# rlglab/minizero

Hardware: AMD Instinct MI355X
Metric: self-play leaf-evals/s (9x9 Go AlphaZero n=400) (higher is better)
Workload: dtype f32; 1 GPU; BASELINE configs[1]: 9x9 Go AlphaZero, n=400, 6 blocks x 64 ch, 256 parallel games per GPU, synthetic fixed-weight net (seed 0), Dirichlet noise + random rotation + softmax-count moves (reference defaults); games_per_gpu=256, actor_num_simulation=400, pipeline_lanes=1, backend=nccl

## Files before the change

minizero_amd/csrc/pool_body.h:

```cpp
#pragma once
#include "pool.h"
#include <cfloat>
#include <climits>

#ifndef MZ_LPROF
#define MZ_LPROF(k)
#endif

namespace mz {

__device__ __forceinline__ float normalizedMean(const PoolView& v, float reward, float mean, float cnt, int player, int bsize, float lo, float hi)
{
    float value = reward + v.gamma * mean;
    if (v.value_rescale) {
        if (bsize < 2) { return 1.0f; }
        value = (value - lo) / (hi - lo);
        value = 2 * value - 1;
        value = value < -1.0f ? -1.0f : value;
        value = value > 1.0f ? 1.0f : value;
    }
    value = (player == v.flipping_player) ? -value : value;
    return (value * cnt - 0.0f) / (cnt + 0.0f);
}

// ... 83 lines not shown
typedef __attribute__((address_space(3))) const float LdsCFloat;
typedef __attribute__((address_space(3))) const double LdsCDbl;
constexpr int kSpecCap = 128;
constexpr int kSpecWay = 4 + 3 * kSpecCap;
constexpr int kGw = 4, kLv = 64 / kGw;
#ifndef MZ_SPEC_WAYS
#define MZ_SPEC_WAYS 16
#endif
constexpr int kSpecWays = MZ_SPEC_WAYS;
#define MZ_SPEC_WAYS_IS(n) static_assert(mz::kSpecWays == (n), "this translation unit sizes its LDS for " #n " remembered paths (pool_body.h MZ_SPEC_WAYS)")
static_assert((kSpecWays & (kSpecWays - 1)) == 0 && kSpecWays >= 2 && kSpecWays <= 64, "a power of two of at most one wave's lanes");
constexpr int kHelpSegs = 3;
constexpr int kHelpHdr = 16;
constexpr int kHelpSeg = kHelpHdr + 4 * kLv;
enum : int {
    kSpecNext = kSpecWays * kSpecWay,
    kSpecPasses = kSpecNext + 1,
    kSpecFound = kSpecNext + 3,
    kSpecLevels = kSpecNext + 5,
    kSpecLastWay = kSpecNext + 6,
    kSpecHelped = kSpecNext + 7,
    kSpecHelp = kSpecNext + 8,
};
constexpr int kSpecWords = kSpecHelp + kHelpSegs * kHelpSeg;
constexpr int kSpecNode = 4, kSpecFc = 4 + kSpecCap, kSpecNc = 4 + 2 * kSpecCap;
struct SpecMem { LdsI32* w; LdsCFloat* bias; LdsCDbl* sqrt; };

struct SpecStage {
    double* sqrt_w;
    float* bias_w;
    int* spec_w;
    __device__ __forceinline__ SpecMem mem(bool walk) const { return SpecMem{walk ? (LdsI32*)spec_w : nullptr, (LdsCFloat*)bias_w, (LdsCDbl*)sqrt_w}; }
    __device__ __forceinline__ float* end() const { return reinterpret_cast<float*>(spec_w + kSpecWords); }
};
template <class View>
__device__ __forceinline__ SpecStage specStage(const View& pv, double* rcp_w, int rcp_n, int tid)
{
    const int tab_n = rcp_n - 2;
    double* sqrt_w = rcp_w + rcp_n;
    float* bias_w = reinterpret_cast<float*>(sqrt_w + tab_n);
    int* spec_w = reinterpret_cast<int*>(bias_w + tab_n + (tab_n & 1));
    for (int i = tid; i < tab_n; i += 512) { sqrt_w[i] = pv.sqrt_tab[i]; bias_w[i] = pv.bias_tab[i]; }
    if (tid < kSpecWays) { spec_w[tid * kSpecWay] = 0; }
    if (tid < 8) { spec_w[kSpecNext + tid] = 0; }
    if (tid < kHelpSegs) { spec_w[kSpecHelp + tid * kHelpSeg] = 0; }
    return SpecStage{sqrt_w, bias_w, spec_w};
}

struct SelectJoin {
    LdsI32* word;
    LdsI32* stats;
    int want, leaf, poll_limit, code;
    int* err;
};

template <bool SPEC = false, bool JOIN = false, class RcpPtr>
__device__ __forceinline__ void selectBody(const PoolView& v, const int* __restrict__ start, int g, int lane, RcpPtr rcp, SpecMem sm = SpecMem{nullptr, nullptr, nullptr}, int serial = 0,
                                           SelectJoin join = SelectJoin{nullptr, nullptr, 0, -1, 0, 0, nullptr})
{
    GNodeRec* recs = (GNodeRec*)(v.rec + size_t(g) * v.cap);
    int* path = v.path + size_t(g) * v.max_depth;
    int* pact = v.path_action + size_t(g) * v.max_depth;
    int* hact = v.host_path_action ? v.host_path_action + size_t(g) * v.max_depth : nullptr;
    MZ_GLOBAL const float* bias_tab = (MZ_GLOBAL const float*)v.bias_tab;
    MZ_GLOBAL const double* sqrt_tab = (MZ_GLOBAL const double*)v.sqrt_tab;
    LdsI32* spec = nullptr;
    auto note = [&](int d, int n, const NodeRec& r) {
        if (!SPEC || !sm.w) { return; }
        if (d == 1) {
            const int w = lane < kSpecWays ? lane : 0;
            const int lw = sm.w[w * kSpecWay], nw = sm.w[w * kSpecWay + kSpecNode + 1];
            const unsigned long long m = __ballot(lane < kSpecWays && lw > 1 && nw == n);
            int way;
            if (m != 0) {
                way = static_cast<int>(__builtin_ctzll(m));
                if (lane == 0) { sm.w[kSpecFound] += 1; }
            } else {
                way = __builtin_amdgcn_readfirstlane(sm.w[kSpecNext]) & (kSpecWays - 1);
                if (lane == 0) { sm.w[kSpecNext] = way + 1; sm.w[way * kSpecWay] = 0; }
            }
            spec = sm.w + way * kSpecWay;
            if (lane == 0) { sm.w[kSpecLastWay] = way; }
        }
        if (spec && lane == 0 && d < kSpecCap) {
            spec[kSpecNode + d] = n;
            spec[kSpecFc + d] = r.first_child;
            spec[kSpecNc + d] = r.num_children;
        }
    };
    const int bsize = v.bound_size[g];
    const float lo = v.bound_lo[g], hi = v.bound_hi[g];
    auto uniformRec = [](NodeRec r) {
        NodeRec u;
        u.count = __int_as_float(__builtin_amdgcn_readfirstlane(__float_as_int(r.count)));
        u.mean = __int_as_float(__builtin_amdgcn_readfirstlane(__float_as_int(r.mean)));
        u.policy = __int_as_float(__builtin_amdgcn_readfirstlane(__float_as_int(r.policy)));
        u.reward = __int_as_float(__builtin_amdgcn_readfirstlane(__float_as_int(r.reward)));
        u.first_child = __builtin_amdgcn_readfirstlane(r.first_child);
        u.num_children = __builtin_amdgcn_readfirstlane(r.num_children);
        u.action = __builtin_amdgcn_readfirstlane(r.action);
        u.players = __builtin_amdgcn_readfirstlane(r.players);
        return u;
    };
    NodeRec cur = uniformRec(loadRec(recs));
    int node = 0, depth = 1;
    if (lane == 0) { path[0] = 0; pact[0] = cur.action; if (hact) { hact[0] = cur.action; } }
    const int st = start ? __builtin_amdgcn_readfirstlane(start[g]) : 0;
    if (st > 0) {
        node = st;
        cur = uniformRec(loadRec(recs + st));
        if (lane == 0) { path[1] = st; pact[1] = cur.action; if (hact) { hact[1] = cur.action; } }
// ... 289 lines not shown
            unsigned long long m = __ballot(vis);
            while (m) { const int j = __builtin_ctzll(m); m &= m - 1; sum_of_win += laneF(q, j); sum += 1; }
        }
        const float init_q = v.atari_init_q ? (sum > 0 ? sum_of_win / sum : 1.0f) : (sum_of_win - 1) / (sum + 1);
        float bs = -FLT_MAX, bp = -FLT_MAX;
        int bi = INT_MAX;
        NodeRec best = c0;
        auto consider = [&](const NodeRec& c, float q, int i) {
            const float bpol = bias * c.policy;
            const float value_u = static_cast<float>((static_cast<double>(bpol) * sqrtN) / static_cast<double>(1 + c.count));
            const float value_q = (c.count == 0.0f) ? init_q : q;
            const float score = value_u + value_q;
            if (better(score, c.policy, i, bs, bp, bi)) { bs = score; bp = c.policy; bi = i; best = c; }
        };
        if (has0) { consider(c0, q0, lane); }
        if (has1) { consider(c1, q1, lane + 64); }
        for (int cb = 128; cb < nc; cb += 64) {
            const int i = cb + lane;
            if (i < nc) {
                const NodeRec c = loadRec(recs + fc + i);
                const float q = (c.count != 0.0f) ? normalizedMean(v, c.reward, c.mean, c.count, cplayer, bsize, lo, hi) : 0.0f;
                consider(c, q, i);
            }
        }
        float rs = bs, rp = bp;
        int ri = bi;
        dppBest<0x111, 0xF>(rs, rp, ri);
        dppBest<0x112, 0xF>(rs, rp, ri);
        dppBest<0x114, 0xF>(rs, rp, ri);
        dppBest<0x118, 0xF>(rs, rp, ri);
        dppBest<0x142, 0xA>(rs, rp, ri);
        dppBest<0x143, 0xC>(rs, rp, ri);
        ri = laneI(ri, 63);
        const int owner = __builtin_ctzll(__ballot(bi == ri));
        cur.count = laneF(best.count, owner);
        cur.first_child = laneI(best.first_child, owner);
        cur.num_children = laneI(best.num_children, owner);
        cur.action = laneI(best.action, owner);
        cur.players = laneI(best.players, owner);
        node = fc + ri;
        note(depth, node, cur);
        if (lane == 0) {
            path[depth] = node;
            pact[depth] = cur.action;
            if (hact) { hact[depth] = cur.action; }
        }
        ++depth;
    }
    if (lane == 0) {
        v.path_len[g] = depth;
        if (v.host_path_len) { v.host_path_len[g] = depth; }
        if (spec) { spec[0] = depth < kSpecCap ? depth : kSpecCap; }
    }
}

template <class RcpPtr>
__device__ __forceinline__ void selectSpecHelper(const PoolView& v, int g, int lane, int seg, int serial, RcpPtr rcp, SpecMem sm)
{
    if (!sm.w || v.atari_init_q || v.value_rescale || seg < 1 || seg > kHelpSegs) { return; }
    LdsI32* out = sm.w + kSpecHelp + (seg - 1) * kHelpSeg;
    const int way = __builtin_amdgcn_readfirstlane(sm.w[kSpecLastWay]) & (kSpecWays - 1);
    LdsI32* spec = sm.w + way * kSpecWay;
    const int plen = __builtin_amdgcn_readfirstlane(spec[0]);
    const int L0 = 1 + seg * kLv, depth = L0 + 1;
    const int max_depth = __builtin_amdgcn_readfirstlane(v.max_depth);
    int adv = 0, n0 = -1;
    int f_count = 0, f_fc = 0, f_nc = 0, f_act = 0, f_pl = 0, f_node = 0;
    if (L0 + 1 < plen && L0 + 1 < kSpecCap) {
        GNodeRec* recs = (GNodeRec*)(v.rec + size_t(g) * v.cap);
        MZ_GLOBAL const float* bias_tab = (MZ_GLOBAL const float*)v.bias_tab;
        MZ_GLOBAL const double* sqrt_tab = (MZ_GLOBAL const double*)v.sqrt_tab;
        int K = plen - L0 < kSpecCap - L0 ? plen - L0 : kSpecCap - L0;
        K = K < kLv ? K : kLv;
        const int k = lane / kGw, j = lane % kGw, Lk = L0 + k, base8 = lane - j;
        const bool inrange = k < K;
        n0 = __builtin_amdgcn_readfirstlane(spec[kSpecNode + L0]);
        const int nk = inrange ? spec[kSpecNode + Lk] : 0;
        const int fck = inrange ? spec[kSpecFc + Lk] : 0;
        const int nck = inrange ? spec[kSpecNc + Lk] : 0;
        const int pfc = (inrange && k >= 1) ? spec[kSpecFc + Lk - 1] : 0;
        const int pnc = (inrange && k >= 1) ? spec[kSpecNc + Lk - 1] : 0;
        const int nl = nck < kGw ? nck : kGw;
        const bool ld = inrange && j < nl && fck >= 0 && fck + j < v.cap;
        const NodeRec c = loadRec(recs + (ld ? fck + j : 0));
        const NodeRec h0 = loadRec(recs + ((n0 >= 0 && n0 < v.cap) ? n0 : 0));
        const int idx = nk - pfc;
        const bool idx_ok = idx >= 0 && idx < kGw && idx < pnc;
        const int srcl = idx_ok ? base8 - kGw + idx : lane;
        float hcount = __shfl(c.count, srcl);
        int hfc = __shfl(c.first_child, srcl), hnc = __shfl(c.num_children, srcl), hpl = __shfl(c.players, srcl);
        if (k == 0) { hcount = h0.count; hfc = h0.first_child; hnc = h0.num_children; hpl = h0.players; }
        bool okk = inrange && ld == (j < nl) && nck > 0 && n0 >= 0 && n0 < v.cap && (k == 0 || idx_ok) && hfc == fck && hnc == nck && hcount >= 1.0f;
        int Nk = static_cast<int>(hcount - 1);
        Nk = okk ? Nk : 0;
        const float biask = sm.bias ? sm.bias[Nk] : bias_tab[Nk];
        const double sqrtNk = sm.sqrt ? sm.sqrt[Nk] : sqrt_tab[Nk];
        const unsigned visn = static_cast<unsigned>(hpl) >> 16;
        const int nek = (visn == 0xFFFFu) ? nck : (nck < static_cast<int>(visn) + 1 ? nck : static_cast<int>(visn) + 1);
        okk = okk && nek <= kGw;
        const int cplk = (hpl >> 8) & 0xFF;
        const bool has = okk && j < nek;
        const RcpPtr rp = rcp + (has ? static_cast<int>(c.count) : 0);
        bool tiny = false;
        const LevelEval e = evalChild(v, c, cplk, biask, sqrtNk, rp[0], rp[1], &tiny);
        const bool vis = has && c.count != 0.0f;
        if (__ballot(vis && tiny) == 0) {
// ... 264 lines not shown
```

minizero_amd/csrc/sim.hip:

```cpp
#include "sim_az_body.h"
#include "sim_mz_body.h"

namespace mz {

MZ_SPEC_WAYS_IS(16);

template <int H, int W, int CIN0_PAD, int CDYN_PAD, int CPAD>
__global__ __launch_bounds__(512) void sim_kernel_mz(const SimArgs* __restrict__ a_, int sim0, int nsims, int host_start, int pre_epoch)
{
    CSimArgs* a = (CSimArgs*)a_;
    extern __shared__ __attribute__((aligned(16))) float tiles[];
    const int g = blockIdx.x, tid = threadIdx.x, lane = tid & 63, wave = tid >> 6;
    constexpr int CM = CIN0_PAD > CDYN_PAD ? (CIN0_PAD > CPAD ? CIN0_PAD : CPAD) : (CDYN_PAD > CPAD ? CDYN_PAD : CPAD);
    constexpr int kTileFloats = kTowerTiles * CM * planeStride(H, W);
    double* rcp_w = reinterpret_cast<double*>(tiles + kTileFloats);
    const int rcp_n = a->rcp_n;
    for (int i = tid; i < rcp_n; i += 512) { rcp_w[i] = a->pv.rcp_tab[i]; }
    LdsCDouble* rcp_lds = (LdsCDouble*)rcp_w;
    const int tab_n = rcp_n - 2;
    double* sqrt_w = rcp_w + rcp_n;
    float* bias_w = reinterpret_cast<float*>(sqrt_w + tab_n);
    int* spec_w = reinterpret_cast<int*>(bias_w + tab_n + (tab_n & 1));
    for (int i = tid; i < tab_n; i += 512) { sqrt_w[i] = a->pv.sqrt_tab[i]; bias_w[i] = a->pv.bias_tab[i]; }
    if (!a->atari) {
// ... 455 lines not shown
#ifdef MZ_SIM_TPROF
    {
        unsigned long long h[64];
        if (hipMemcpyFromSymbol(h, HIP_SYMBOL(g_tp), sizeof(h)) == hipSuccess && h[63]) {
            fprintf(stderr, "[mz sim tprof] cycles per layer (game 0, avg over %llu towers):", h[63]);
            for (int i = 0; i < 14; ++i) { fprintf(stderr, " %.0f", double(h[i]) / double(h[63])); }
            fprintf(stderr, "\n");
        }
    }
#endif
    if (sim_prof_.n == 0) { return; }
    hipLaunchKernelGGL(sim_prof_fold, dim3(1), dim3(1), 0, stream_, sim_prof_.p + sim_prof_.n - kSimProfTail);
    if (hipStreamSynchronize(stream_) != hipSuccess) { return; }
    std::vector<unsigned long long> h(sim_prof_.n);
    if (hipMemcpy(h.data(), sim_prof_.p, h.size() * sizeof(unsigned long long), hipMemcpyDeviceToHost) != hipSuccess) { return; }
    const std::vector<unsigned long long> tail(h.end() - kSimProfTail, h.end());
    h.resize(h.size() - kSimProfTail);
    double skipped = 0, skipped_max = 0, sims_all = 0;
    for (size_t g = 0; g < h.size() / 8; ++g) {
        const double sk = double(h[g * 8 + 4] >> 32);
        h[g * 8 + 4] &= 0xFFFFFFFFull;
        skipped += sk; sims_all += double(h[g * 8 + 4]);
        skipped_max = std::max(skipped_max, sk / std::max(1.0, double(h[g * 8 + 4])));
    }
    { double ps = 0, ac = 0, kk = 0; for (size_t g = 0; g < h.size() / 8; ++g) { ps += double(h[g * 8 + 7] >> 40); ac += double((h[g * 8 + 7] >> 20) & 0xFFFFF); kk += double(h[g * 8 + 7] & 0xFFFFF); } fprintf(stderr, "[mz sim prof] path speculation: %.0f passes, %.0f levels taken, %.0f walks that found a remembered path\n", ps, ac, kk); }
    const char* names[4] = {"select+leaf", "tower", "heads", "cand+expand"};
    const size_t G = h.size() / 8;
    double tot_all = 0, tot_max = 0;
    for (int k = 0; k < 4; ++k) {
        double sum = 0, mx = 0, sims = 0;
        for (size_t g = 0; g < G; ++g) { sum += double(h[g * 8 + k]); mx = std::max(mx, double(h[g * 8 + k])); sims += double(h[g * 8 + 4]); }
        fprintf(stderr, "[mz sim prof] %-12s avg %8.2f us per simulation (slowest game %8.2f us)\n", names[k], sum / std::max(1.0, sims) * 0.01,
                mx / std::max(1.0, sims / G) * 0.01);
        tot_all += sum / std::max(1.0, sims) * 0.01;
    }
    {
        double sel = 0, lev = 0, sims = 0, maxlev = 0;
        double helped = 0;
        const unsigned long long low = (1ull << 40) - 1;
        for (size_t g = 0; g < G; ++g) { sel += double(h[g * 8 + 5]); lev += double(h[g * 8 + 6] & low); helped += double(h[g * 8 + 6] >> 40); sims += double(h[g * 8 + 4]); maxlev = std::max(maxlev, double(h[g * 8 + 6] & low) / std::max(1.0, double(h[g * 8 + 4]))); }
        fprintf(stderr, "[mz sim prof] levels taken over from the helper waves: %.0f (%.1f %% of all levels)\n", helped, 100.0 * helped / std::max(1.0, lev));
        fprintf(stderr, "[mz sim prof] select alone avg %8.2f us, path length avg %.2f (deepest game avg %.2f) -> %.2f us per level\n", sel / std::max(1.0, sims) * 0.01,
                lev / std::max(1.0, sims), maxlev, sel / std::max(1.0, lev) * 0.01);
    }
    for (size_t g = 0; g < G; ++g) { tot_max = std::max(tot_max, double(h[g * 8] + h[g * 8 + 1] + h[g * 8 + 2] + h[g * 8 + 3]) / std::max(1.0, double(h[g * 8 + 4])) * 0.01); }
    fprintf(stderr, "[mz sim prof] total        avg %8.2f us per simulation (slowest game %8.2f us)\n", tot_all, tot_max);
    {
        double tw = 0, hd = 0;
        for (size_t g = 0; g < G; ++g) { tw += double(h[g * 8 + 1]); hd += double(h[g * 8 + 2]); }
        const double ran = std::max(1.0, sims_all - skipped);
        fprintf(stderr, "[mz sim prof] terminal leaves: network skipped in %.0f of %.0f simulations (%.2f %%; the game with the most: %.2f %%) -> per simulation that ran them: tower %.2f us, heads %.2f us\n",
                skipped, sims_all, 100.0 * skipped / std::max(1.0, sims_all), 100.0 * skipped_max, tw / ran * 0.01, hd / ran * 0.01);
    }
    fprintf(stderr, "[mz sim prof] heads ahead: %llu of the %.0f simulations that ran the network used the heads with their operands delivered ahead\n", tail[7],
            sims_all - skipped);
    fprintf(stderr, "[mz sim prof] value first: %llu of %.0f simulations in the new order; %llu walks arrived at the previous simulation's leaf, %llu waited there (avg %.2f us); "
                    "%llu waits at the join in front of the leaf\n",
            tail[16], sims_all, tail[17], tail[18], double(tail[19]) / std::max(1.0, double(tail[18])) * 0.01, tail[20]);
    if (tail[8] > 0) {
        const double L = double(tail[8]), first = double(tail[9]) / L * 0.01, last = double(tail[10]) / L * 0.01, mean = double(tail[11]) / L * 0.01;
        const double helping = double(tail[12]) / L * 0.01;
        fprintf(stderr, "[mz sim prof] launches: %llu, avg per launch from the first game's start: first game done %.1f us, mean %.1f us, last %.1f us -> %.1f %% of the CU time idles at the end of a launch\n",
                tail[8], first, mean, last, 100.0 * (last - mean - helping) / std::max(1e-9, last));
        if (tail[13] > 0 || tail[15] > 0 || tail[21] > 0) {
            double tw = 0;
            for (size_t g = 0; g < G; ++g) { tw += double(h[g * 8 + 1]); }
            const double ran = sims_all - skipped, qn = double(tail[21]), qt = double(tail[22]), pn = double(tail[13]) + qn, pt = double(tail[14]) + qt;
            const double ln = double(tail[33]), lt = double(tail[34]);
            fprintf(stderr, "[mz sim prof] tail help: %.0f of the %.0f simulations that ran the network had a pair tower (%.2f %%): tower %.2f us with a helper, %.2f us alone; %llu games helped, "
                            "a CU helps for %.1f us per launch after its own game (%.1f %% of the launch)\n",
                    pn, ran, 100.0 * pn / std::max(1.0, ran), pt / std::max(1.0, pn) * 0.01, (tw - pt - lt) / std::max(1.0, ran - pn - ln) * 0.01, tail[15], helping,
                    100.0 * helping / std::max(1e-9, last));
            fprintf(stderr, "[mz sim prof] tail help, quad towers: %.0f of the %.0f simulations that ran the network had a quad tower (%.2f %%): tower %.2f us with three helpers, %.2f us with "
                            "one; %llu games went from pair to quad towers\n",
                    qn, ran, 100.0 * qn / std::max(1.0, ran), qt / std::max(1.0, qn) * 0.01, (pt - qt) / std::max(1.0, pn - qn) * 0.01, tail[23]);
            const double ia = double(tail[30]) / L * 0.01, ib = double(tail[31]) / L * 0.01, ic = double(tail[32]) / L * 0.01;
            fprintf(stderr, "[mz sim prof] tail help, idle CU time by the reason the CU stopped looking for a game to help (%% of the launch): (a) every running game of its XCD had its "
                            "helpers %.2f %%, (b) no game of its XCD was running any more %.2f %%, (c) only games with fewer than help_min_left simulations were left %.2f %%\n",
                    100.0 * ia / std::max(1e-9, last), 100.0 * ib / std::max(1e-9, last), 100.0 * ic / std::max(1e-9, last));
        }
        if (tail[33] > 0 || tail[35] > 0 || tail[36] > 0) {
            const double ran = sims_all - skipped, ln = double(tail[33]), taken = double(tail[35]);
            fprintf(stderr, "[mz sim prof] lending: %.0f of the %.0f simulations that ran the network had a tower lent by a game that was ahead (%.2f %%): tower %.2f us with the volunteer; "
                            "%llu offers taken, %llu of them withdrawn behind a terminal leaf, %llu taken too late; a volunteer waits %.2f us for its command and is away for %.2f us per "
                            "offer taken, %.1f us per launch and CU (%.1f %% of the launch)\n",
                    ln, ran, 100.0 * ln / std::max(1.0, ran), double(tail[34]) / std::max(1.0, ln) * 0.01, tail[35], tail[37], tail[36], double(tail[38]) / std::max(1.0, taken) * 0.01,
                    double(tail[39]) / std::max(1.0, taken) * 0.01, double(tail[39]) / std::max(1.0, double(G)) / L * 0.01, 100.0 * double(tail[39]) / std::max(1.0, double(G)) / L * 0.01 / std::max(1e-9, last));
        }
    }
}

static size_t simLdsBound(size_t tile_bytes, int n, int A, size_t head_floats)
{
    const size_t rcp_n = size_t(n) + 5, max_depth = size_t(n) + 3;
    return tile_bytes + rcp_n * (2 * sizeof(double) + sizeof(float)) + kSpecWords * sizeof(int) + (size_t(5) * (A + 1) + 26 + 18 * 12 + 2 * max_depth + 2 + head_floats) * sizeof(float) +
           size_t(kGoSeenCap) * sizeof(uint64_t);
}

int Net::uploadSimArgs(const SimArgs& a)
{
    static_assert(sizeof(SimArgs) % 4 == 0, "SimArgs is copied as words");
    if (sim_args_host_.size() != sizeof(SimArgs) || memcmp(sim_args_host_.data(), &a, sizeof(SimArgs)) != 0) {
        if (!sim_args_.ensure(sizeof(SimArgs))) { setError("hipMalloc of the simulation arguments failed"); return MZ_ERR_DEVICE; }
        MZ_HIP(hipStreamSynchronize(stream_));
        MZ_HIP(hipMemcpy(sim_args_.p, &a, sizeof(SimArgs), hipMemcpyHostToDevice));
        sim_args_host_.assign(reinterpret_cast<const char*>(&a), reinterpret_cast<const char*>(&a) + sizeof(SimArgs));
// ... 416 lines not shown
```

minizero_amd/csrc/sim_az_body.h:

```cpp
#pragma once
#include "net.h"
#ifdef MZ_SIM_TPROF
__device__ unsigned long long g_tp[64];
__shared__ unsigned long long s_tp_prev;
__shared__ int s_tp_idx;
#define MZ_TPROF(slot)                                                                         \
    do {                                                                                       \
        if ((slot) == 3 && threadIdx.x == 0 && blockIdx.x == 0) {                              \
            const unsigned long long t_ = clock64();                                           \
            g_tp[s_tp_idx & 63] += t_ - s_tp_prev; s_tp_prev = t_; ++s_tp_idx;                 \
        }                                                                                      \
    } while (0)
#endif
#ifdef MZ_SIM_HPROF
#ifndef MZ_HPROF_BLOCK
#define MZ_HPROF_BLOCK 0
#endif
__device__ unsigned long long g_hp[16];
__shared__ unsigned long long s_hp_prev;
#define MZ_HPROF(k)                                                                                   \
    do {                                                                                              \
        if (threadIdx.x == 0 && blockIdx.x == MZ_HPROF_BLOCK) {                                       \
            const unsigned long long t_ = wall_clock64();                                             \
            if ((k) > 0) { g_hp[(k)] += t_ - s_hp_prev; } else { g_hp[15] += 1; }                     \
// ... 194 lines not shown
}

template <int WPE>
__device__ __forceinline__ void simCandExpandImpl(CSimArgs* __restrict__ a, int rot, int slot, int g, int lane, float* tiles, float* xchg, int part)
{
    g = __builtin_amdgcn_readfirstlane(g);
    slot = __builtin_amdgcn_readfirstlane(slot);
    rot = __builtin_amdgcn_readfirstlane(rot);
    const GoDevView gv = simLeafView(ldc(&a->gv), xchg, g);
    const PoolView pv = simPathView(ldc(&a->pv), reinterpret_cast<int*>(xchg) - 2 * a->pv.max_depth - 2, g);
    const SimXchg x{gv.A + (gv.A & 1)};
    const size_t ga = size_t(g) * gv.A;
    float* sc = xchg + x.scalars();
    int* cand_count = reinterpret_cast<int*>(sc + 1) - g;
    int* cand_player = reinterpret_cast<int*>(sc + 2) - g;
    int* cand_action = reinterpret_cast<int*>(xchg + x.caction()) - ga;
    Cand* cs = reinterpret_cast<Cand*>(tiles);
    Cand* out = cs + gv.A;
    const int k = reinterpret_cast<const int*>(sc)[1];
    if (a->cand_coop == 2) {
        if (k > 0 && k <= kCandCoopMaxW) {
            float* dense = simCandDense(tiles, gv.A);
            candScatterW(cs, out, reinterpret_cast<int*>(out + gv.A), k, 8, lane, reinterpret_cast<const int*>(dense + kCandCoopMaxW), a->err);
        }
    } else if (k > 0 && k <= kCandCoopMax && a->cand_coop) {
        float* dense = simCandDense(tiles, gv.A);
        candScatter(cs, out, reinterpret_cast<int*>(out + gv.A), k, 8, lane, reinterpret_cast<const int*>(dense + kCandCoopMax), a->err);
    }
    MZ_LPROF(8);
    azCandStore(gv, sc - g, out, k, cand_count, cand_action, xchg + x.cpolicy() - ga, xchg + x.clogit() - ga, cand_player, sc + 3 - g, sc + 4 - g, g, lane);
    waveSync();
    MZ_LPROF(9);
    expandBackupBody(pv, cand_count, cand_action, xchg + x.cpolicy() - ga, xchg + x.clogit() - ga, cand_player, sc + 3 - g, sc + 4 - g, slot, a->err, g,
                     lane, tiles, part);
    MZ_LPROF(12);
}

template <int WPE>
__device__ __noinline__ void simCandExpand(CSimArgs* __restrict__ a, int rot, int slot, int g, int lane, float* tiles, float* xchg, int part)
{
    simCandExpandImpl<WPE>(a, rot, slot, g, lane, tiles, xchg, part);
}

constexpr int kVfBackup = 4;
constexpr int kVfLeaf = 5;
constexpr int kVfGather = 7;
constexpr int kVfRank = 8;
constexpr int kVfExpand = 9;
constexpr int kVfStats = 10;
constexpr int kVfWalked = 14;
constexpr int kVfOffer = 15;
constexpr int kVfLend = 16;
constexpr int kVfLendStat = 18;
constexpr int kVfLendBits = 24;
constexpr int kVfWords = kVfLendBits + 3 * kHpMaxUnits;
constexpr int kVfErr = 97;

__device__ __forceinline__ bool vfWait(LdsI32* w, int want, int* err, int lane)
{
    int seen = __builtin_amdgcn_readfirstlane(__hip_atomic_load(w, __ATOMIC_RELAXED, __HIP_MEMORY_SCOPE_WORKGROUP));
    const bool waited = seen < want;
    for (int i = 0; i < kHpPollLimit && seen < want; ++i) {
        __builtin_amdgcn_s_sleep(1);
        seen = __builtin_amdgcn_readfirstlane(__hip_atomic_load(w, __ATOMIC_RELAXED, __HIP_MEMORY_SCOPE_WORKGROUP));
    }
    if (seen < want && lane == 0) { atomicExch(err, kVfErr); }
    __builtin_amdgcn_fence(__ATOMIC_ACQUIRE, "workgroup");
    return waited;
}
__device__ __forceinline__ void vfPublish(LdsI32* w, int serial, int lane)
{
    __builtin_amdgcn_fence(__ATOMIC_RELEASE, "workgroup");
    __builtin_amdgcn_wave_barrier();
    if (lane == 0) { __hip_atomic_store(w, serial, __ATOMIC_RELAXED, __HIP_MEMORY_SCOPE_WORKGROUP); }
}

template <class RcpPtr>
__device__ __noinline__ void simWalkVf(CSimArgs* __restrict__ a, int g, int lane, RcpPtr rcp, SpecMem spec, float* xchg, int serial, int join_leaf, int join_want, int* vf_)
{
    serial = __builtin_amdgcn_readfirstlane(serial);
    g = __builtin_amdgcn_readfirstlane(g);
    join_leaf = __builtin_amdgcn_readfirstlane(join_leaf);
    join_want = __builtin_amdgcn_readfirstlane(join_want);
    LdsI32* vf = (LdsI32*)vf_;
    unsigned long long t0 = 0;
    if (a->prof) { t0 = wall_clock64(); }
    const PoolView pv = simPathView(ldc(&a->pv), reinterpret_cast<int*>(xchg) - 2 * a->pv.max_depth - 2, g);
    selectBody<true, true>(pv, nullptr, g, lane, rcp, spec, serial, SelectJoin{vf + kVfExpand, vf + kVfStats, join_want, join_leaf, kHpPollLimit, kVfErr, a->err});
    waveSync();
    if (a->prof && lane == 0) {
        a->prof[size_t(g) * 8 + 5] += wall_clock64() - t0;
        a->prof[size_t(g) * 8 + 6] += pv.path_len[g];
    }
}

template <int CPL>
__device__ __noinline__ void simLeafVf(CSimArgs* __restrict__ a, int rot, int slot, int g, int lane, float* xchg, const uint64_t* seen_lds, uint64_t* leaf_smem, int* vf)
{
    g = __builtin_amdgcn_readfirstlane(g);
    slot = __builtin_amdgcn_readfirstlane(slot);
    rot = __builtin_amdgcn_readfirstlane(rot);
    if constexpr (CPL > 0) {
        const PoolView pv = simPathView(ldc(&a->pv), reinterpret_cast<int*>(xchg) - 2 * a->pv.max_depth - 2, g);
        const GoDevView gv = simLeafView(ldc(&a->gv), xchg, g);
        if (lane == 0) {
            const int len = pv.path_len[g];
            vf[kVfLeaf] = len > 0 ? (pv.path + size_t(g) * pv.max_depth)[len - 1] : 0;
            vf[kVfLeaf + 1] = len > 0 ? 1 : 0;
        }
        leafBody<CPL, true, 1>(gv, pv, rot, slot, g, lane, leaf_smem, seen_lds);
    }
}

template <int WPE>
__device__ __noinline__ void simCandPipeVf(CSimArgs* __restrict__ a, int rot, int slot, int g, int lane, int w, int serial, float* tiles, float* xchg, int* vf_)
{
    g = __builtin_amdgcn_readfirstlane(g);
    w = __builtin_amdgcn_readfirstlane(w);
    serial = __builtin_amdgcn_readfirstlane(serial);
    LdsI32* vf = (LdsI32*)vf_;
    const int A = a->gv.A;
    const SimXchg x{A + (A & 1)};
    if (w == 0) {
        simCandGatherImpl<WPE>(a, rot, g, lane, tiles, xchg);
        vfPublish(vf + kVfGather, serial, lane);
    } else {
        vfWait(vf + kVfGather, serial, a->err, lane);
    }
    const int k = __builtin_amdgcn_readfirstlane(reinterpret_cast<const int*>(xchg + x.scalars())[1]);
    float* dense = simCandDense(tiles, A);
    if (k > 0 && k <= kCandCoopMax && a->cand_coop) {
        candRankPart(dense, k, w, 8, lane, reinterpret_cast<int*>(dense + kCandCoopMax));
        candRankPart(dense, k, w + 4, 8, lane, reinterpret_cast<int*>(dense + kCandCoopMax));
    }
    if (w != 0) {
        __builtin_amdgcn_fence(__ATOMIC_RELEASE, "workgroup");
        __builtin_amdgcn_wave_barrier();
        if (lane == 0) { __hip_atomic_fetch_add(vf + kVfRank, 1, __ATOMIC_RELAXED, __HIP_MEMORY_SCOPE_WORKGROUP); }
        return;
    }
    vfWait(vf + kVfRank, 3 * serial, a->err, lane);
    slot = __builtin_amdgcn_readfirstlane(slot);
    const GoDevView gv = simLeafView(ldc(&a->gv), xchg, g);
    PoolView pv = simPathView(ldc(&a->pv), reinterpret_cast<int*>(xchg) - 2 * a->pv.max_depth - 2, g);
    pv.path = vf_ + kVfLeaf - size_t(g) * pv.max_depth;
    pv.path_len = vf_ + kVfLeaf + 1 - g;
    const size_t ga = size_t(g) * gv.A;
    float* sc = xchg + x.scalars();
    int* cand_count = reinterpret_cast<int*>(sc + 1) - g;
    int* cand_player = reinterpret_cast<int*>(sc + 2) - g;
    int* cand_action = reinterpret_cast<int*>(xchg + x.caction()) - ga;
    Cand* cs = reinterpret_cast<Cand*>(tiles);
    Cand* out = cs + gv.A;
    if (k > 0 && k <= kCandCoopMax && a->cand_coop) { candScatter(cs, out, reinterpret_cast<int*>(out + gv.A), k, 8, lane, reinterpret_cast<const int*>(dense + kCandCoopMax), a->err); }
    azCandStore(gv, sc - g, out, k, cand_count, cand_action, xchg + x.cpolicy() - ga, xchg + x.clogit() - ga, cand_player, sc + 3 - g, sc + 4 - g, g, lane);
    waveSync();
    expandBackupBody(pv, cand_count, cand_action, xchg + x.cpolicy() - ga, xchg + x.clogit() - ga, cand_player, sc + 3 - g, sc + 4 - g, slot, a->err, g, lane, tiles, 1);
    vfPublish(vf + kVfExpand, serial, lane);
}

template <int WPE>
__device__ __noinline__ void simApplyRootNoise(CSimArgs* __restrict__ a, int g, int lane)
{
    g = __builtin_amdgcn_readfirstlane(g);
    const PoolView v = ldc(&a->pv);
    const size_t base = size_t(g) * v.cap;
    const int nc = v.rec[base].num_children;
    const size_t fc = base + v.rec[base].first_child;
    const float eps = a->noise_eps;
    for (int i = lane; i < nc; i += 64) {
        const float nz = a->root_noise[size_t(g) * v.A + i];
        if (a->noise_kind == kNoiseDirichlet) { v.rec[fc + i].policy = (1 - eps) * v.rec[fc + i].policy + eps * nz; }
        else { v.logit[fc + i] = v.logit[fc + i] + nz; }
        v.noise[fc + i] = nz;
    }
    waveSync();
}

template <int WPE>
__device__ __noinline__ void simGumbelStart(CSimArgs* __restrict__ a, int slot, bool host_start, int g, int lane, float* tiles, int* state_lds = nullptr)
{
    g = __builtin_amdgcn_readfirstlane(g);
    slot = __builtin_amdgcn_readfirstlane(slot);
    if (host_start && slot >= 1) { return; }
    int st = 0;
    if (slot >= 1 && !host_start) {
        const PoolView pv = ldc(&a->pv);
        GumbelView gum = ldc(&a->gum);
        if (state_lds) { gum.state = state_lds - size_t(g) * (3 + kGumbelMaxSample); }
        st = gumbelStepBody(pv, gum, slot, g, lane, tiles);
    }
    if (lane == 0) { a->start[g] = st; }
    waveSync();
}

template <int WPE, bool BIGA = false, bool FP = BIGA>
__device__ __forceinline__ void simHeadsImpl(CSimArgs* __restrict__ a, int g, int tid, float* tiles, const float* xtile, int xcs, int xpw, float* xchg)
{
    g = __builtin_amdgcn_readfirstlane(g);
    xcs = __builtin_amdgcn_readfirstlane(xcs);
    xpw = __builtin_amdgcn_readfirstlane(xpw);
    MZ_HPROF(0);
    const HeadParams hp = ldc(&a->hp);
    const SimXchg x{hp.A + (hp.A & 1)};
    const size_t ga = size_t(g) * hp.A;
    headsBody<BIGA, FP>(nullptr, hp, xchg + x.policy() - ga, xchg + x.logit() - ga, xchg + x.scalars() - g, nullptr, nullptr, 0, g, tid, 512, tiles, xtile, xcs, xpw);
    MZ_HPROF(1);
}
template <int WPE, bool BIGA = false, bool FP = BIGA>
__device__ __noinline__ void simHeads(CSimArgs* __restrict__ a, int g, int tid, float* tiles, const float* xtile, int xcs, int xpw, float* xchg)
{
    simHeadsImpl<WPE, BIGA, FP>(a, g, tid, tiles, xtile, xcs, xpw, xchg);
}

template <int H, int W>
__device__ __forceinline__ void simHeadsAhead(CSimArgs* __restrict__ a, int tid, float* tiles, const float* xtile, float* xchg, const float* hw)
{
    MZ_HPROF(0);
    const HeadParams hp = ldc(&a->hp);
    const SimXchg x{HeadsAhead::A + (HeadsAhead::A & 1)};
    headsBodyAhead<planeStride(H, W), W + 2>(hp, xchg + x.policy(), xchg + x.logit(), xchg + x.scalars(), tid, tiles, xtile, hw);
    MZ_HPROF(1);
}

__device__ __forceinline__ bool simLeafTerminal(CSimArgs* __restrict__ a, const float* xchg)
{
    if (a->no_spec & 16) { return false; }
    const int A = a->gv.A;
    const SimXchg x{A + (A & 1)};
    return __builtin_amdgcn_readfirstlane(reinterpret_cast<const int*>(xchg + x.scalars())[6]) != 0;
}

constexpr int kSimProfTail = 40;
__device__ __forceinline__ void simProfEnter(unsigned long long* tail)
{
    atomicMin(tail + 0, wall_clock64() - tail[4]);
}
__device__ __forceinline__ void simProfExit(unsigned long long* tail)
{
    const unsigned long long t = wall_clock64() - tail[4];
    atomicMin(tail + 1, t);
    atomicMax(tail + 2, t);
    atomicAdd(tail + 3, t);
    atomicAdd(tail + 5, 1ull);
}
__device__ __forceinline__ void simProfSim(unsigned long long* prof, unsigned long long t0, unsigned long long t1, unsigned long long t2, unsigned long long t3, unsigned long long t4,
                                           bool term = false)
{
    prof[0] += t1 - t0 + (term ? t3 - t1 : 0); prof[1] += term ? 0 : t2 - t1; prof[2] += term ? 0 : t3 - t2; prof[3] += t4 - t3;
    prof[4] += 1 + (static_cast<unsigned long long>(term) << 32);
}
__device__ __forceinline__ void simProfSpec(unsigned long long* prof, const int* spec_w)
{
    prof[7] += (static_cast<unsigned long long>(spec_w[kSpecPasses]) << 40) | (static_cast<unsigned long long>(spec_w[kSpecLevels]) << 20) | spec_w[kSpecFound];
    prof[6] += static_cast<unsigned long long>(spec_w[kSpecHelped]) << 40;
}

template <int H, int W, int CIN0_PAD, int CPAD, bool BF = false>
constexpr int simWavesPerEu() { return (!BF && H * W <= 64 && kTowerTiles * (CIN0_PAD > CPAD ? CIN0_PAD : CPAD) * planeStride(H, W) * 4 <= 76 * 1024) ? 4 : 2; }
template <int H, int W, int CIN0_PAD, int CPAD, bool BF>
constexpr int simTileFloats() { return BF ? towerBf16LdsBytes<H, W>(true) / 4 : kTowerTiles * (CIN0_PAD > CPAD ? CIN0_PAD : CPAD) * planeStride(H, W); }

template <int H, int W, int CIN0_PAD, int CPAD>
__device__ __noinline__ const float* simTower(CSimArgs* __restrict__ a, int g, int tid, float* tiles, float* xchg)
{
    g = __builtin_amdgcn_readfirstlane(g);
#ifdef MZ_SIM_TPROF
    if (tid == 0 && g == 0) { s_tp_prev = clock64(); s_tp_idx = 0; g_tp[63] += 1; }
#endif
    g = __builtin_amdgcn_readfirstlane(g);
    const GoDevView gv = simLeafView(ldc(&a->gv), xchg, g);
    return towerBody<H, W, CIN0_PAD, CPAD>(reinterpret_cast<const float*>(gv.feat), a->params, *(const TowerArgs*)&a->ta, nullptr, g, tid, tiles);
}

template <int H, int W>
__device__ __noinline__ const float* simTowerBf16(CSimArgs* __restrict__ a, int g, int tid, float* tiles, float* xchg)
{
    g = __builtin_amdgcn_readfirstlane(g);
    const GoDevView gv = simLeafView(ldc(&a->gv), xchg, g);
    return towerBodyBf16<H, W>(reinterpret_cast<const unsigned*>(gv.feat), a->wfrag, a->params, *(const TowerArgsBf16*)&a->tb, nullptr, g, tid,
                               reinterpret_cast<char*>(tiles));
}

template <int H, int W, int CIN0_PAD, int CPAD, int MODE>
__device__ __forceinline__ const float* simTowerHelped(CSimArgs* __restrict__ a, int g, int tid, float* tiles, float* xchg, int seq, unsigned xseq, int* abort_lds, bool lent = false)
{
    g = __builtin_amdgcn_readfirstlane(g);
    seq = __builtin_amdgcn_readfirstlane(seq);
    xseq = __builtin_amdgcn_readfirstlane(xseq);
    const GoDevView gv = simLeafView(ldc(&a->gv), xchg, g);
    const unsigned* bits = reinterpret_cast<const unsigned*>(gv.feat) + size_t(g) * gv.channels * gv.W32;
    unsigned* hb = a->help + size_t(g) * a->help_words;
    const int fw = gv.channels * gv.W32;
    if (tid < helpCmdUnits(fw)) {
        hpu4 u;
        u.x = bits[3 * tid];
        u.y = 3 * tid + 1 < fw ? bits[3 * tid + 1] : 0u;
        u.z = 3 * tid + 2 < fw ? bits[3 * tid + 2] : 0u;
        u.w = hpCmdWord(unsigned(seq), MODE, xseq, lent);
        asm volatile("global_store_dwordx4 %0, %1, off" ::"v"(hb + kHpCmd + 4 * tid), "v"(u) : "memory");
    }
    HelpCtx c{hb, 0, xseq, abort_lds, a->err, tiles + a->pair_slot};
    if constexpr (MODE == kHpModeQuad) { return towerBodyQuad<H, W, CIN0_PAD, CPAD>(bits, a->params, *(const TowerArgs*)&a->ta, tid, tiles, c); }
// ... 310 lines not shown
    unsigned long long pair_n = 0, pair_t = 0;
    unsigned long long quad_n = 0, quad_t = 0;
    unsigned long long lent_n = 0, lent_t = 0;
    unsigned long long lend_t = 0;
    if (help_on && tid == 0) { s_help[0] = 0; s_help[1] = 0; hpStoreU(help_blk + kHpXcc, hpXccId()); }
    bool vf = false;
    if constexpr (kHelp) {
        vf = leaf_smem != nullptr && !a->use_gumbel && !a->pv.value_rescale && a->cand_coop != 2 && !(a->no_spec & 64);
        if (tid >= kVfBackup && tid < kVfWords) { s_help[tid] = 0; }
    }
    unsigned long long vf_t0 = 0, vf_n = 0;
    const bool lend_on = kHelp && help_on && vf && !(a->no_spec & 256);
    __syncthreads();
    for (int s = 0; s < nsims; ++s) {
        const int slot = sim0 + s;
        const int rot = rot_tab[size_t(s) * games + g];
        unsigned long long t0 = 0, t1 = 0, t2 = 0, t3 = 0, t4 = 0;
        if (prof) { t0 = (vf && s > 0) ? vf_t0 : wall_clock64(); }
        if (kHelp && vf) {
            if constexpr (kHelp) {
                if (wave == 0) {
                    if (s == 0) {
                        if (slot == 1 && a->root_noise) { simApplyRootNoise<WPE>(a, g, lane); }
                        simWalkVf(a, g, lane, rcp_lds, spec, xchg, (a->no_spec & 2) ? 0 : 1, -1, 0, s_help);
                        if (lend_on && lane == 0) { __hip_atomic_store((LdsI32*)s_help + kVfWalked, 1, __ATOMIC_RELAXED, __HIP_MEMORY_SCOPE_WORKGROUP); }
                    } else {
                        const bool waited = vfWait((LdsI32*)s_help + kVfExpand, s, a->err, lane);
                        if (prof && waited && lane == 0) { s_help[kVfStats + 3] += 1; }
                        if (help_on && lane == 0) { hpStoreU(help_blk + kHpProgress, unsigned(s)); }
                    }
                    simLeafVf<CPL>(a, rot, slot, g, lane, xchg, seen_lds, leaf_smem, s_help);
                } else if (s == 0 && wave <= kHelpSegs && spec.w && !(a->no_spec & 2)) {
                    simSelectHelper(a, g, lane, wave, 1, rcp_lds, spec);
                } else if (lend_on && wave == 7) {
                    simLendScan(a, g, lane, s, nsims, help_blk, s_help);
                } else if (help_on && tid == 7 * 64) {
                    s_help[1] = simHelpMode(help_blk);
                }
            }
        } else if (wave == 0) {
            if (slot == 1 && a->root_noise) { simApplyRootNoise<WPE>(a, g, lane); }
            if (a->use_gumbel) { simGumbelStart<WPE>(a, slot, s == 0 && (host_start & 1) != 0, g, lane, tiles); }
            simSelectLeaf<CPL, WPE>(a, rot, slot, g, lane, tiles, rcp_lds, spec, xchg, seen_lds, (a->no_spec & 2) ? 0 : s + 1, leaf_smem);
        } else if (WPE == 2 && wave <= kHelpSegs && spec.w && !(a->no_spec & 2)) {
            simSelectHelper(a, g, lane, wave, s + 1, rcp_lds, spec);
        } else if (kHelp && help_on && tid == 7 * 64) {
            s_help[1] = simHelpMode(help_blk);
        }
        __syncthreads();
        const int help_mode = (kHelp && help_on) ? __builtin_amdgcn_readfirstlane(s_help[1]) : 0;
        const bool lent = lend_on && __builtin_amdgcn_readfirstlane(s_help[kVfOffer]) != 0;
        const bool pair = help_mode == 1 || lent, quad = help_mode == 2;
        const bool term = simLeafTerminal(a, xchg);
        if constexpr (kHelp) {
            if (lend_on) {
                if (lent && term && tid == 7 * 64) { hpStoreU(help_blk + kHpOffer, 0u); }
                const int lend_to = __builtin_amdgcn_readfirstlane(s_help[kVfLend]);
                if (lend_to != 0) {
                    const unsigned long long tl0 = prof ? wall_clock64() : 0;
                    if (!simLendTower<H, W, CIN0_PAD, CPAD>(a, lend_to - 1, __builtin_amdgcn_readfirstlane(s_help[kVfLend + 1]), tid, tiles, s_help)) { return; }
                    if (prof) { const unsigned long long d = wall_clock64() - tl0; t0 += d; lend_t += d; }
                }
            }
        }
        if constexpr (CPL > 0) {
            if (!term) {
                simLeafPlanes<CPL>(a, rot, g, wave, lane, leaf_smem ? leaf_smem : reinterpret_cast<const uint64_t*>(tiles), xchg);
                __syncthreads();
            }
        }
        if (prof) { t1 = wall_clock64(); }
        const float* xt = nullptr;
        if (!term) {
            if constexpr (BF) { xt = simTowerBf16<H, W>(a, g, tid, tiles, xchg); }
            else if constexpr (WPE == 4) {
                const GoDevView gvt = simLeafView(ldc(&a->gv), xchg, g);
                xt = towerBody<H, W, CIN0_PAD, CPAD>(reinterpret_cast<const float*>(gvt.feat), a->params, *(const TowerArgs*)&a->ta, nullptr, g, tid, tiles);
            }
            else if constexpr (kHelp) {
                if (pair) {
                    xt = simTowerPair<H, W, CIN0_PAD, CPAD>(a, g, tid, tiles, xchg, s + 1, help_xseq, s_help, lent ? 1 : 0);
                    if (!xt) { return; }
                    help_xseq += unsigned(a->ta.nlayers);
                    if (lent && tid == 7 * 64) { hpStoreU(help_blk + kHpOffer, 0u); }
                }
                else if (quad) {
                    xt = simTowerQuad<H, W, CIN0_PAD, CPAD>(a, g, tid, tiles, xchg, s + 1, help_xseq, s_help);
                    if (!xt) { return; }
                    help_xseq += unsigned(a->ta.nlayers);
                }
                else { xt = simTower<H, W, CIN0_PAD, CPAD>(a, g, tid, tiles, xchg); }
            }
            else { xt = simTower<H, W, CIN0_PAD, CPAD>(a, g, tid, tiles, xchg); }
        }
        __syncthreads();
        if (prof) { t2 = wall_clock64(); }
        if constexpr (WPE == 4) { if (!term) { simHeadsImpl<WPE>(a, g, tid, tiles, xt, planeStride(H, W), W + 2, xchg); } }
        else if (leaf_smem && wave >= 6) { simLeafRest<CPL>(a, rot, slot, g, lane, xchg, seen_lds, leaf_smem, 7 - wave); }
        else if (!term) {
            bool ahead = false;
            if constexpr (kAhead) { ahead = heads_w != nullptr; }
            if (ahead) { if constexpr (kAhead) { simHeadsAhead<H, W>(a, tid, tiles, xt, xchg, heads_w); } }
            else { simHeads<WPE, false, (MZ_HEADS_FP != 0)>(a, g, tid, tiles, xt, planeStride(H, W), W + 2, xchg); }
        }
        else if (leaf_smem) { __syncthreads(); __syncthreads(); }
        __syncthreads();
        if (prof) { t3 = wall_clock64(); }
        if (kHelp && vf) {
            if constexpr (kHelp) {
                const bool more = s + 1 < nsims;
                if (wave == 0) {
                    simBackupOnly<WPE>(a, slot, g, lane, tiles, xchg);
                    vfPublish((LdsI32*)s_help + kVfBackup, s + 1, lane);
                    if (prof && tid == 0) {
                        t4 = wall_clock64();
                        simProfSim(prof, t0, t1, t2, t3, t4, term);
                        if (pair && !lent && !term) { pair_n += 1; pair_t += t2 - t1; }
                        if (quad && !term) { quad_n += 1; quad_t += t2 - t1; }
                        if (lent && !term) { lent_n += 1; lent_t += t2 - t1; }
                        if constexpr (kAhead) { if (heads_w && !term) { ahead_n += 1; } }
                        vf_n += 1;
                    }
                    vf_t0 = t4;
                    if (more) {
                        if (slot + 1 == 1 && a->root_noise) {
                            vfWait((LdsI32*)s_help + kVfExpand, s + 1, a->err, lane);
                            simApplyRootNoise<WPE>(a, g, lane);
                        }
                        simWalkVf(a, g, lane, rcp_lds, spec, xchg, (a->no_spec & 2) ? 0 : s + 2, __builtin_amdgcn_readfirstlane(s_help[kVfLeaf]), s + 1, s_help);
                        if (lend_on && lane == 0) { __hip_atomic_store((LdsI32*)s_help + kVfWalked, s + 2, __ATOMIC_RELAXED, __HIP_MEMORY_SCOPE_WORKGROUP); }
                    }
                } else if (wave <= kHelpSegs) {
                    if (more && spec.w && !(a->no_spec & 2)) {
                        vfWait((LdsI32*)s_help + kVfBackup, s + 1, a->err, lane);
                        simSelectHelper(a, g, lane, wave, s + 2, rcp_lds, spec);
                    }
                } else {
                    simCandPipeVf<WPE>(a, rot, slot, g, lane, wave - 4, s + 1, tiles, xchg, s_help);
                }
            }
            continue;
        }
        if (wave == 0) { simCandGather<WPE>(a, rot, g, lane, tiles, xchg); }
        __syncthreads();
        {
            const int A = a->gv.A;
            const SimXchg x{A + (A & 1)};
            if (a->cand_coop) { simCandRank(A, reinterpret_cast<const int*>(xchg + x.scalars())[1], wave, lane, tiles); }
        }
        __syncthreads();
        {
            const bool split = !a->pv.value_rescale;
            if (wave == 0) { simCandExpand<WPE>(a, rot, slot, g, lane, tiles, xchg, split ? 1 : 0); }
            else if (wave == 1 && split) { simBackupOnly<WPE>(a, slot, g, lane, tiles, xchg); }
        }
        __syncthreads();
        if (prof && tid == 0) {
            t4 = wall_clock64();
            simProfSim(prof, t0, t1, t2, t3, t4, term);
            if (pair && !term) { pair_n += 1; pair_t += t2 - t1; }
            if (quad && !term) { quad_n += 1; quad_t += t2 - t1; }
            if constexpr (kAhead) { if (heads_w && !term) { ahead_n += 1; } }
        }
        if (kHelp && help_on && tid == 0) { hpStoreU(help_blk + kHpProgress, unsigned(s) + 1u); }
    }
    if constexpr (kHelp) {
        if (vf) {
            __syncthreads();
            if (help_on && tid == 0) { hpStoreU(help_blk + kHpProgress, unsigned(nsims)); }
            if (prof && tid == 0) {
                unsigned long long* ptail = a->prof + size_t(games) * 8;
                atomicAdd(ptail + 16, vf_n);
                for (int i = 0; i < 4; ++i) { atomicAdd(ptail + 17 + i, static_cast<unsigned long long>(s_help[kVfStats + i])); }
                if (lend_on) {
// ... 28 lines not shown
```

Measured before the change: 1.771 million leaf-evals/s.

## Answer revisited terminal leaves from the tree instead of replaying the leaf

When the value-first walk ends at a node already visited with no children (a terminal found earlier), the leaf stage now skips the game replay and terminal check. It sets the terminal flag, leaf player and stored value directly, and the backup runs without touching the history slot. The intent is to remove repeated leaf simulation for terminal positions that MCTS revisits often late in games. It adds profiling counters and a verification re-run under profiling, and it relies on count>0 with zero children meaning terminal, which could misfire if an expanded node can have zero children for another reason.

```diff
diff --git a/minizero_amd/csrc/pool_body.h b/minizero_amd/csrc/pool_body.h
--- a/minizero_amd/csrc/pool_body.h
+++ b/minizero_amd/csrc/pool_body.h
@@ -159,11 +159,12 @@
     LdsI32* stats;
     int want, leaf, poll_limit, code;
     int* err;
+    LdsI32* end = nullptr;
 };
 
 template <bool SPEC = false, bool JOIN = false, class RcpPtr>
 __device__ __forceinline__ void selectBody(const PoolView& v, const int* __restrict__ start, int g, int lane, RcpPtr rcp, SpecMem sm = SpecMem{nullptr, nullptr, nullptr}, int serial = 0,
-                                           SelectJoin join = SelectJoin{nullptr, nullptr, 0, -1, 0, 0, nullptr})
+                                           SelectJoin join = SelectJoin{nullptr, nullptr, 0, -1, 0, 0, nullptr, nullptr})
 {
     GNodeRec* recs = (GNodeRec*)(v.rec + size_t(g) * v.cap);
     int* path = v.path + size_t(g) * v.max_depth;
@@ -559,6 +560,9 @@
         if (v.host_path_len) { v.host_path_len[g] = depth; }
         if (spec) { spec[0] = depth < kSpecCap ? depth : kSpecCap; }
     }
+    if constexpr (JOIN) {
+        if (join.end && lane == 0) { join.end[0] = (cur.count > 0.0f && cur.num_children == 0) ? 1 : 0; }
+    }
 }
 
 template <class RcpPtr>
diff --git a/minizero_amd/csrc/sim.hip b/minizero_amd/csrc/sim.hip
--- a/minizero_amd/csrc/sim.hip
+++ b/minizero_amd/csrc/sim.hip
@@ -531,6 +531,15 @@
         fprintf(stderr, "[mz sim prof] terminal leaves: network skipped in %.0f of %.0f simulations (%.2f %%; the game with the most: %.2f %%) -> per simulation that ran them: tower %.2f us, heads %.2f us\n",
                 skipped, sims_all, 100.0 * skipped / std::max(1.0, sims_all), 100.0 * skipped_max, tw / ran * 0.01, hd / ran * 0.01);
     }
+    if (tail[16] > 0) {
+        const double first_n = double(tail[42]), rev_n = double(tail[44]), term_n = first_n + rev_n, ans = double(tail[40]);
+        fprintf(stderr, "[mz sim prof] terminal revisits: %llu of %.0f terminal simulations answered from the tree (%.2f %%); %llu arrived at a leaf already found terminal; "
+                        "part 1 re-run under the profile disagreed in %llu\n",
+                tail[40], term_n, 100.0 * ans / std::max(1.0, term_n), tail[44], tail[41]);
+        fprintf(stderr, "[mz sim prof] terminal simulation, previous backup to own backup: first visit avg %.2f us (%llu), revisit avg %.2f us (%llu; of which %.2f us the "
+                        "profile's own re-run of part 1)\n",
+                double(tail[43]) / std::max(1.0, first_n) * 0.01, tail[42], double(tail[45]) / std::max(1.0, rev_n) * 0.01, tail[44], double(tail[46]) / std::max(1.0, rev_n) * 0.01);
+    }
     fprintf(stderr, "[mz sim prof] heads ahead: %llu of the %.0f simulations that ran the network used the heads with their operands delivered ahead\n", tail[7],
             sims_all - skipped);
     fprintf(stderr, "[mz sim prof] value first: %llu of %.0f simulations in the new order; %llu walks arrived at the previous simulation's leaf, %llu waited there (avg %.2f us); "
diff --git a/minizero_amd/csrc/sim_az_body.h b/minizero_amd/csrc/sim_az_body.h
--- a/minizero_amd/csrc/sim_az_body.h
+++ b/minizero_amd/csrc/sim_az_body.h
@@ -270,6 +270,7 @@
 constexpr int kVfOffer = 15;
 constexpr int kVfLend = 16;
 constexpr int kVfLendStat = 18;
+constexpr int kVfWalkEnd = 22;
 constexpr int kVfLendBits = 24;
 constexpr int kVfWords = kVfLendBits + 3 * kHpMaxUnits;
 constexpr int kVfErr = 97;
@@ -304,13 +305,17 @@
     unsigned long long t0 = 0;
     if (a->prof) { t0 = wall_clock64(); }
     const PoolView pv = simPathView(ldc(&a->pv), reinterpret_cast<int*>(xchg) - 2 * a->pv.max_depth - 2, g);
-    selectBody<true, true>(pv, nullptr, g, lane, rcp, spec, serial, SelectJoin{vf + kVfExpand, vf + kVfStats, join_want, join_leaf, kHpPollLimit, kVfErr, a->err});
+    selectBody<true, true>(pv, nullptr, g, lane, rcp, spec, serial, SelectJoin{vf + kVfExpand, vf + kVfStats, join_want, join_leaf, kHpPollLimit, kVfErr, a->err, vf + kVfWalkEnd});
     waveSync();
     if (a->prof && lane == 0) {
         a->prof[size_t(g) * 8 + 5] += wall_clock64() - t0;
         a->prof[size_t(g) * 8 + 6] += pv.path_len[g];
     }
 }
+
+constexpr int kVfRevisit = 1;
+constexpr int kVfRevWrong = 2;
+constexpr int kVfRevArrived = 4;
 
 template <int CPL>
 __device__ __noinline__ void simLeafVf(CSimArgs* __restrict__ a, int rot, int slot, int g, int lane, float* xchg, const uint64_t* seen_lds, uint64_t* leaf_smem, int* vf)
@@ -321,13 +326,46 @@
     if constexpr (CPL > 0) {
         const PoolView pv = simPathView(ldc(&a->pv), reinterpret_cast<int*>(xchg) - 2 * a->pv.max_depth - 2, g);
         const GoDevView gv = simLeafView(ldc(&a->gv), xchg, g);
+        const SimXchg x{gv.A + (gv.A & 1)};
+        int* sci = reinterpret_cast<int*>(xchg + x.scalars());
+        const int len = __builtin_amdgcn_readfirstlane(pv.path_len[g]);
+        const int leaf = len > 0 ? __builtin_amdgcn_readfirstlane((pv.path + size_t(g) * pv.max_depth)[len - 1]) : 0;
         if (lane == 0) {
-            const int len = pv.path_len[g];
-            vf[kVfLeaf] = len > 0 ? (pv.path + size_t(g) * pv.max_depth)[len - 1] : 0;
+            vf[kVfLeaf] = leaf;
             vf[kVfLeaf + 1] = len > 0 ? 1 : 0;
         }
-        leafBody<CPL, true, 1>(gv, pv, rot, slot, g, lane, leaf_smem, seen_lds);
-    }
+        const bool arrived = len > 0 && __builtin_amdgcn_readfirstlane(vf[kVfWalkEnd]) != 0;
+        const bool answer = arrived && !(a->no_spec & (1024 | 16));
+        unsigned long long tc = 0;
+        if (answer && a->prof) { tc = wall_clock64(); }
+        if (!answer || a->prof) { leafBody<CPL, true, 1>(gv, pv, rot, slot, g, lane, leaf_smem, seen_lds); }
+        if (answer) {
+            int state = kVfRevisit | kVfRevArrived, ticks = 0;
+            if (a->prof) {
+                waveSync();
+                if (__builtin_amdgcn_readfirstlane(gv.terminal[g]) == 0) { state |= kVfRevWrong; }
+                ticks = static_cast<int>(wall_clock64() - tc);
+            }
+            if (lane == 0) {
+                const int root_turn = gv.snap[g].turn;
+                gv.leaf_player[g] = ((len - 1) & 1) ? 3 - root_turn : root_turn;
+                gv.terminal[g] = 1;
+                gv.eval[g] = pv.value[size_t(g) * pv.cap + leaf];
+                sci[10] = state;
+                sci[11] = ticks;
+            }
+        } else if (lane == 0) {
+            sci[10] = arrived ? kVfRevArrived : 0;
+            sci[11] = 0;
+        }
+    }
+}
+
+__device__ __forceinline__ int simLeafRevisit(CSimArgs* __restrict__ a, const float* xchg)
+{
+    const int A = a->gv.A;
+    const SimXchg x{A + (A & 1)};
+    return __builtin_amdgcn_readfirstlane(reinterpret_cast<const int*>(xchg + x.scalars())[10]);
 }
 
 template <int WPE>
@@ -373,7 +411,8 @@
     if (k > 0 && k <= kCandCoopMax && a->cand_coop) { candScatter(cs, out, reinterpret_cast<int*>(out + gv.A), k, 8, lane, reinterpret_cast<const int*>(dense + kCandCoopMax), a->err); }
     azCandStore(gv, sc - g, out, k, cand_count, cand_action, xchg + x.cpolicy() - ga, xchg + x.clogit() - ga, cand_player, sc + 3 - g, sc + 4 - g, g, lane);
     waveSync();
-    expandBackupBody(pv, cand_count, cand_action, xchg + x.cpolicy() - ga, xchg + x.clogit() - ga, cand_player, sc + 3 - g, sc + 4 - g, slot, a->err, g, lane, tiles, 1);
+    const int hslot = (__builtin_amdgcn_readfirstlane(reinterpret_cast<const int*>(sc)[10]) & kVfRevisit) ? -1 : slot;
+    expandBackupBody(pv, cand_count, cand_action, xchg + x.cpolicy() - ga, xchg + x.clogit() - ga, cand_player, sc + 3 - g, sc + 4 - g, hslot, a->err, g, lane, tiles, 1);
     vfPublish(vf + kVfExpand, serial, lane);
 }
 
@@ -449,7 +488,7 @@
     return __builtin_amdgcn_readfirstlane(reinterpret_cast<const int*>(xchg + x.scalars())[6]) != 0;
 }
 
-constexpr int kSimProfTail = 40;
+constexpr int kSimProfTail = 48;
 __device__ __forceinline__ void simProfEnter(unsigned long long* tail)
 {
     atomicMin(tail + 0, wall_clock64() - tail[4]);
@@ -467,6 +506,15 @@
 {
     prof[0] += t1 - t0 + (term ? t3 - t1 : 0); prof[1] += term ? 0 : t2 - t1; prof[2] += term ? 0 : t3 - t2; prof[3] += t4 - t3;
     prof[4] += 1 + (static_cast<unsigned long long>(term) << 32);
+}
+__device__ __forceinline__ void simProfTerminal(unsigned long long* tail, const float* sc, unsigned long long ticks)
+{
+    const int state = reinterpret_cast<const int*>(sc)[10], check = reinterpret_cast<const int*>(sc)[11];
+    unsigned long long* w = tail + ((state & kVfRevArrived) ? 44 : 42);
+    atomicAdd(w, 1ull);
+    atomicAdd(w + 1, ticks);
+    if (state & kVfRevisit) { atomicAdd(tail + 40, 1ull); atomicAdd(tail + 46, static_cast<unsigned long long>(check)); }
+    if (state & kVfRevWrong) { atomicAdd(tail + 41, 1ull); }
 }
 __device__ __forceinline__ void simProfSpec(unsigned long long* prof, const int* spec_w)
 {
@@ -883,6 +931,8 @@
         const bool lent = lend_on && __builtin_amdgcn_readfirstlane(s_help[kVfOffer]) != 0;
         const bool pair = help_mode == 1 || lent, quad = help_mode == 2;
         const bool term = simLeafTerminal(a, xchg);
+        bool revisit = false;
+        if constexpr (kHelp) { revisit = vf && term && (simLeafRevisit(a, xchg) & kVfRevisit) != 0; }
         if constexpr (kHelp) {
             if (lend_on) {
                 if (lent && term && tid == 7 * 64) { hpStoreU(help_blk + kHpOffer, 0u); }
@@ -927,7 +977,10 @@
         __syncthreads();
         if (prof) { t2 = wall_clock64(); }
         if constexpr (WPE == 4) { if (!term) { simHeadsImpl<WPE>(a, g, tid, tiles, xt, planeStride(H, W), W + 2, xchg); } }
-        else if (leaf_smem && wave >= 6) { simLeafRest<CPL>(a, rot, slot, g, lane, xchg, seen_lds, leaf_smem, 7 - wave); }
+        else if (leaf_smem && wave >= 6) {
+            if (revisit) { __syncthreads(); __syncthreads(); }
+            else { simLeafRest<CPL>(a, rot, slot, g, lane, xchg, seen_lds, leaf_smem, 7 - wave); }
+        }
         else if (!term) {
             bool ahead = false;
             if constexpr (kAhead) { ahead = heads_w != nullptr; }
@@ -951,6 +1004,7 @@
                         if (lent && !term) { lent_n += 1; lent_t += t2 - t1; }
                         if constexpr (kAhead) { if (heads_w && !term) { ahead_n += 1; } }
                         vf_n += 1;
+                        if (term) { simProfTerminal(a->prof + size_t(games) * 8, xchg + SimXchg{a->gv.A + (a->gv.A & 1)}.scalars(), t4 - t0); }
                     }
                     vf_t0 = t4;
                     if (more) {
```

Result: no change. 1.777 million leaf-evals/s, median of 6 (+0.3%).
